# data61/stellar-random-walk

Measured on AMD Instinct MI355X. Metric: walk-steps/sec, higher is better.
Workload: dtype f64

## Files before the change

### include/stellar_rw.h

```cpp
#ifndef STELLAR_RW_H
#define STELLAR_RW_H
#include <stddef.h>
#include <stdint.h>

#ifdef __cplusplus
extern "C" {
#endif

typedef struct srw_handle srw_handle;

enum {
  SRW_OK = 0,
  SRW_ERR_INVALID = 1,
  SRW_ERR_IO = 2,
  SRW_ERR_PARSE = 3,
  SRW_ERR_HIP = 4,
  SRW_ERR_EXISTS = 5,
  SRW_ERR_NOMEM = 6
};

enum {
  SRW_SAMPLER_REFERENCE = 0,
  SRW_SAMPLER_ALIAS = 1
};
enum {
  SRW_RNG_CONST = 0,
  SRW_RNG_PHILOX = 1
};

typedef struct {
  int32_t device;
  int32_t rank;
  int32_t world;
  int32_t flags;
} srw_config;
enum {
  SRW_CFG_OWNER_FROM_PARTITIONS = 1,
  SRW_CFG_COMPACT_IDS = 2,
  SRW_CFG_NO_MEMBERSHIP = 4,
  SRW_CFG_OWNER_HASH_PARTITIONER = 8
};

int32_t srw_create(const srw_config *cfg, srw_handle **out);
void srw_destroy(srw_handle *h);
const char *srw_last_error(const srw_handle *h);
int32_t srw_set_stream(srw_handle *h, void *hip_stream);

int32_t srw_plan_walks(srw_handle *h, int64_t num_walks);

int32_t srw_load_edgelist(srw_handle *h, const char *path, int32_t directed, int32_t weighted,
                          int32_t partitioned, int32_t rdd_partitions);
int32_t srw_load_coo(srw_handle *h, const int32_t *src, const int32_t *dst, const float *w,
                     const int32_t *pid, int64_t n_lines, int32_t directed);
enum { SRW_IDS_I32 = 0, SRW_IDS_I64 = 1 };
int32_t srw_load_coo_device(srw_handle *h, const void *d_src, const void *d_dst, const float *d_w,
                            int64_t n_lines, int32_t id_type, int32_t directed);
int32_t srw_load_adjacency(srw_handle *h, const int32_t *vids, const int64_t *offs, int64_t n_rows,
                           const int32_t *ids, const float *w, const int32_t *pids);
int32_t srw_generate_rmat(srw_handle *h, int32_t scale, int64_t n_edges, uint32_t seed, int32_t weighted,
                          int32_t directed);

int32_t srw_graph_stats(const srw_handle *h, int64_t *n_vertices, int64_t *n_entries);
int32_t srw_graph_vertices(const srw_handle *h, int32_t *out);
int32_t srw_graph_neighbors(const srw_handle *h, int32_t v, int32_t *ids, float *w, int64_t cap, int64_t *n);
int32_t srw_graph_partition(const srw_handle *h, int32_t v, int32_t *pid, int32_t *known);

typedef struct {
  float p, q;
  int32_t walk_length;
  int32_t num_walks;
  int32_t first_walk;
  int32_t rng_mode;
  float const_r;
  uint32_t seed;
  int32_t sampler;
  int32_t flags;
} srw_walk_params;
enum {
  SRW_WALK_FORCE_GENERAL = 1,
  SRW_WALK_NT_LOADS = 2,
  SRW_WALK_CACHED_LOADS = 4,
  SRW_WALK_NO_COMPACT = 16,
  SRW_WALK_NO_PREFIX = 32,
  SRW_WALK_NO_EDGE_HASH = 64,
  SRW_WALK_NO_BINNED = 128,
  SRW_WALK_DEVICE_FORMAT = 131072,
  SRW_WALK_NO_HUB_BITMAPS = 65536,
  SRW_WALK_NO_EDGE_TABLES = 262144,
  SRW_WALK_EDGE_TABLES_ALL = 524288
};

typedef struct {
  int64_t n_walkers;
  int64_t n_steps;
  int64_t dead_ends;
  int64_t sum_deg_curr;
  int64_t sum_deg_prev;
  int64_t ent_reads;
  int64_t fallbacks;
  int64_t trials;
  double kernel_ms;
  int32_t kernel_kind;
  int32_t record_bytes;
  int64_t strategy_steps[12];
  int64_t edge_tables;
  int64_t edge_table_bytes;
  double setup_ms;
} srw_walk_stats;
enum {
  SRW_STRAT_EDGE_TABLE = 0,
  SRW_STRAT_P1 = 1,
  SRW_STRAT_P2 = 2,
  SRW_STRAT_W = 3,
  SRW_STRAT_P3 = 4,
  SRW_STRAT_SCAN = 5,
  SRW_STRAT_PREFIX = 6,
  SRW_STRAT_CHAIN = 7,
  SRW_STRAT_EDGE_MASK = 8,
  SRW_STRAT_Q1_LANE = 9,
  SRW_STAT_HANDED_OVER = 10,
  SRW_STAT_TIES_RESOLVED = 11
};

int32_t srw_walk(srw_handle *h, const srw_walk_params *params, srw_walk_stats *stats);
int32_t srw_walk_to_host(srw_handle *h, const srw_walk_params *params, int32_t *paths, int32_t *lens,
                         srw_walk_stats *stats);
int32_t srw_walk_and_save(srw_handle *h, const srw_walk_params *params, const char *output_dir, int32_t n_parts,
                          int32_t write_crc, srw_walk_stats *stats, int64_t *dead_ends_per_iteration);
int32_t srw_set_sources(srw_handle *h, const int32_t *ids, int64_t n);
int32_t srw_set_sources_device(srw_handle *h, const void *d_ids, int64_t n);
int32_t srw_clear_sources(srw_handle *h);
int32_t srw_sources(const srw_handle *h, int64_t *n);

int32_t srw_vertex_types_set(srw_handle *h, const void *d_types, int64_t n);
int32_t srw_vertex_types(const srw_handle *h, int64_t *n);
int32_t srw_walk_metapath(srw_handle *h, const srw_walk_params *params, const int32_t *pattern, int32_t m, srw_walk_stats *stats);

typedef struct { uint32_t seed; uint32_t epoch; int32_t replace; int32_t flags; } srw_neighbor_params;
enum { SRW_NBR_NO_COMPACT = 1  };
int32_t srw_sample_neighbors(srw_handle *h, const void *d_seeds , int64_t n_seeds,
                             const int32_t *fanouts , int32_t n_layers, const srw_neighbor_params *np,
                             void *const *d_layers , int64_t *n_unknown );

int32_t srw_host_alloc(size_t bytes, void **out);
void srw_host_free(void *p);
int32_t srw_fetch_paths(const srw_handle *h, int32_t *paths, int32_t *lens);
int32_t srw_device_paths(const srw_handle *h, void **d_paths, void **d_lens, int64_t *n_walkers, int32_t *stride);
int32_t srw_write_paths(const srw_handle *h, const char *output_dir, int32_t n_parts, int32_t write_crc);

int32_t srw_alias_row(srw_handle *h, int32_t v, float *prob, int32_t *alias, int64_t cap, int64_t *n, int32_t *regular);

typedef struct {
  int32_t lw;
  int32_t src;
  int32_t prev, curr;
} srw_walker;
typedef struct {
  int32_t lw;
  int32_t v;
} srw_path_ret;
typedef struct { int64_t cap_walkers, cap_rets, chunk_bytes; } srw_shard_layout;
int32_t srw_shard_capacity(const srw_handle *h, int64_t *n_local_vertices, int64_t *n_global_vertices);
int32_t srw_shard_vertex_ranks(const srw_handle *h, int32_t *out);
int32_t srw_shard_layout_for(const srw_handle *h, int32_t batch, double slack, srw_shard_layout *out);
// ... 104 lines not shown
```

### stellar-random-walk_amd/__init__.py

```python
import ctypes as C
import os

import numpy as np

_DIR = os.path.dirname(os.path.abspath(__file__))
LIB_PATH = os.environ.get("SRW_LIB") or os.path.join(_DIR, "libstellar_rw.so")
CLI_PATH = os.path.join(_DIR, "stellar-rw")

OK, ERR_INVALID, ERR_IO, ERR_PARSE, ERR_HIP, ERR_EXISTS, ERR_NOMEM = range(7)
SAMPLER_REFERENCE, SAMPLER_ALIAS = 0, 1
RNG_CONST, RNG_PHILOX = 0, 1
CFG_OWNER_FROM_PARTITIONS = 1
CFG_COMPACT_IDS = 2
CFG_NO_MEMBERSHIP = 4
CFG_OWNER_HASH_PARTITIONER = 8
IDS_I32, IDS_I64 = 0, 1
WALK_FORCE_GENERAL = 1
WALK_NT_LOADS = 2
WALK_CACHED_LOADS = 4
WALK_NO_COMPACT = 16
WALK_NO_PREFIX = 32
WALK_NO_EDGE_HASH = 64
WALK_NO_BINNED = 128
WALK_NO_HUB_BITMAPS = 65536
WALK_DEVICE_FORMAT = 131072
WALK_NO_EDGE_TABLES = 262144
WALK_EDGE_TABLES_ALL = 524288
NBR_NO_COMPACT = 1
NBR_MAX_LAYERS, NBR_MAX_FANOUT, NBR_MAX_DISTINCT_FANOUT = 8, 4096, 64


class W2vParams(C.Structure):
    _fields_ = [("dim", C.c_int32), ("window", C.c_int32), ("iterations", C.c_int32), ("learning_rate", C.c_float),
                ("seed", C.c_uint32), ("threads", C.c_int32)]


def w2v_save(vocab_ids, vectors, output_dir, n_parts=1):
    ids = np.ascontiguousarray(vocab_ids, dtype=np.int32); vec = np.ascontiguousarray(vectors, dtype=np.float32)
    rc = lib().srw_w2v_save(_i32(ids), _f32(vec), len(ids), vec.shape[1] if vec.ndim == 2 else 1, os.fsencode(output_dir), n_parts)
    if rc != 0:
        raise SrwError(rc, "srw_w2v_save: %s" % lib().srw_last_error(None).decode())


class SkipgramParams(C.Structure):
    _fields_ = [("context", C.c_int32), ("num_negatives", C.c_int32), ("seed", C.c_uint32), ("epoch", C.c_uint32)]


class SkipgramBatchParams(C.Structure):
    _fields_ = [("context", C.c_int32), ("num_negatives", C.c_int32), ("seed", C.c_uint32), ("epoch", C.c_uint32),
                ("exclude_window", C.c_int32), ("max_draws", C.c_int32)]


class SgnsParams(C.Structure):
    _fields_ = [("context", C.c_int32), ("num_negatives", C.c_int32), ("dim", C.c_int32), ("center", C.c_int32),
                ("lr", C.c_float), ("reserved", C.c_int32)]


class TopkParams(C.Structure):
    _fields_ = [("dim", C.c_int32), ("k", C.c_int32), ("metric", C.c_int32), ("reserved", C.c_int32)]


TOPK_METRICS = {"cosine": 0, "dot": 1}


class NeighborParams(C.Structure):
    _fields_ = [("seed", C.c_uint32), ("epoch", C.c_uint32), ("replace", C.c_int32), ("flags", C.c_int32)]


class SrwError(RuntimeError):
    def __init__(self, code, msg):
        super().__init__("srw error %d: %s" % (code, msg))
        self.code = code


class Config(C.Structure):
    _fields_ = [("device", C.c_int32), ("rank", C.c_int32), ("world", C.c_int32), ("flags", C.c_int32)]


class WalkParams(C.Structure):
    _fields_ = [("p", C.c_float), ("q", C.c_float), ("walk_length", C.c_int32), ("num_walks", C.c_int32),
                ("first_walk", C.c_int32), ("rng_mode", C.c_int32), ("const_r", C.c_float), ("seed", C.c_uint32),
                ("sampler", C.c_int32), ("flags", C.c_int32)]


class WalkStats(C.Structure):
    _fields_ = [("n_walkers", C.c_int64), ("n_steps", C.c_int64), ("dead_ends", C.c_int64),
                ("sum_deg_curr", C.c_int64), ("sum_deg_prev", C.c_int64), ("ent_reads", C.c_int64),
                ("fallbacks", C.c_int64), ("trials", C.c_int64), ("kernel_ms", C.c_double), ("kernel_kind", C.c_int32),
                ("record_bytes", C.c_int32), ("strategy_steps", C.c_int64 * 12), ("edge_tables", C.c_int64),
                ("edge_table_bytes", C.c_int64), ("setup_ms", C.c_double)]

    def as_dict(self):
        d = {k: getattr(self, k) for k, _ in self._fields_}
        d["strategy_steps"] = dict(zip(STRATEGIES, list(self.strategy_steps)))
        return d


class ShardLayout(C.Structure):
    _fields_ = [("cap_walkers", C.c_int64), ("cap_rets", C.c_int64), ("chunk_bytes", C.c_int64)]


STRATEGIES = ("edge_table", "p1", "p2", "w", "p3", "scan", "prefix", "chain", "edge_mask", "q1_lane", "handed_over_walkers", "ties_resolved")
# ... 333 lines not shown

    def shard_capacity(self):
        a, b = C.c_int64(0), C.c_int64(0)
        self._ck(lib().srw_shard_capacity(self.h, C.byref(a), C.byref(b)))
        return a.value, b.value

    def vertices(self):
        n = self.shard_capacity()[0]
        out = np.zeros(max(n, 1), dtype=np.int32)
        self._ck(lib().srw_graph_vertices(self.h, _i32(out)))
        return out[:n]

    def neighbors(self, v):
        n = C.c_int64(0)
        self._ck(lib().srw_graph_neighbors(self.h, v, None, None, 0, C.byref(n)))
        if n.value < 0:
            return None
        ids = np.zeros(max(n.value, 1), dtype=np.int32)
        w = np.zeros(max(n.value, 1), dtype=np.float32)
        self._ck(lib().srw_graph_neighbors(self.h, v, _i32(ids), _f32(w), n.value, C.byref(n)))
        return ids[:n.value], w[:n.value]

    def partition(self, v):
        pid, known = C.c_int32(0), C.c_int32(0)
        self._ck(lib().srw_graph_partition(self.h, v, C.byref(pid), C.byref(known)))
        return pid.value if known.value else None

    def alias_row(self, v):
        n, reg = C.c_int64(0), C.c_int32(0)
        self._ck(lib().srw_alias_row(self.h, v, None, None, 0, C.byref(n), C.byref(reg)))
        if n.value < 0:
            return None
        prob = np.zeros(max(n.value, 1), dtype=np.float32)
        alias = np.zeros(max(n.value, 1), dtype=np.int32)
        self._ck(lib().srw_alias_row(self.h, v, _f32(prob), _i32(alias), n.value, C.byref(n), C.byref(reg)))
        return reg.value, prob[:n.value], alias[:n.value]

    def set_sources(self, ids):
        if hasattr(ids, "data_ptr") and hasattr(ids, "is_cuda"):
            if "int32" not in str(ids.dtype) or ids.dim() != 1 or not ids.is_contiguous():
                raise TypeError("set_sources: a tensor of ids must be one-dimensional, int32 and contiguous (got %s)" % ids.dtype)
            if ids.is_cuda:
                import torch
                torch.cuda.current_stream(ids.device).synchronize()
                self._ck(lib().srw_set_sources_device(self.h, C.c_void_p(ids.data_ptr()), int(ids.numel())))
                self._src_ids = ids.clone()
                return self
            ids = ids.numpy()
        a = np.asarray(ids)
        if a.size and a.dtype.kind not in "iu":
            raise TypeError("set_sources: vertex ids must be integers (got %s)" % a.dtype)
        if a.size and (int(a.min()) < -2**31 or int(a.max()) > 2**31 - 1):
            raise ValueError("set_sources: a vertex id is outside int32")
        a = np.array(a.reshape(-1), dtype=np.int32)
        self._ck(lib().srw_set_sources(self.h, _i32(a) if a.size else None, a.size))
        self._src_ids = a
        return self

    def clear_sources(self):
        self._ck(lib().srw_clear_sources(self.h))
        self._src_ids = None
        return self

    def sources_len(self):
        n = C.c_int64(0)
        self._ck(lib().srw_sources(self.h, C.byref(n)))
        return None if n.value < 0 else n.value

    def _with_sources(self, sources, call):
        if sources is None:
            return call()
        before = getattr(self, "_src_ids", None) if self.sources_len() is not None else None
        self.set_sources(sources)
        try:
            return call()
        finally:
            if before is None:
                self.clear_sources()
            else:
                self.set_sources(before)

    @staticmethod
    def params(p=1.0, q=1.0, walk_length=80, num_walks=1, first_walk=0, rng="philox", const_r=0.0, seed=42,
               sampler=SAMPLER_REFERENCE, force_general=False, nt_loads=None, occ=0, compact=True, prefix=True, edge_hash=True, binned=True, binned_tune=0, hub_bitmaps=True, device_format=False, edge_tables=True, edge_tables_all=False):
        if sampler == "alias":
            sampler = SAMPLER_ALIAS
        elif sampler == "reference":
            sampler = SAMPLER_REFERENCE
        return WalkParams(np.float32(p), np.float32(q), walk_length, num_walks, first_walk,
                          RNG_CONST if rng == "const" else RNG_PHILOX, np.float32(const_r), seed, sampler,
                          (WALK_FORCE_GENERAL if force_general else 0) | (0 if nt_loads is None else WALK_NT_LOADS if nt_loads else WALK_CACHED_LOADS) | (occ << 8) | (0 if compact else WALK_NO_COMPACT) | (0 if prefix else WALK_NO_PREFIX) | (0 if edge_hash else WALK_NO_EDGE_HASH) | (0 if binned else WALK_NO_BINNED) | (0 if hub_bitmaps else WALK_NO_HUB_BITMAPS) | (WALK_DEVICE_FORMAT if device_format else 0) | (binned_tune << 12) | (0 if edge_tables else WALK_NO_EDGE_TABLES) | (WALK_EDGE_TABLES_ALL if edge_tables_all else 0))

    def walk(self, fetch=True, sources=None, **kw):
        if sources is not None:
            return self._with_sources(sources, lambda: self.walk(fetch=fetch, **kw))
        P = self.params(**kw)
        st = WalkStats()
        self._ck(lib().srw_walk(self.h, C.byref(P), C.byref(st)))
        if not fetch:
            return st.as_dict()
        paths = np.empty((max(st.n_walkers, 1), P.walk_length + 2), dtype=np.int32)
        lens = np.empty(max(st.n_walkers, 1), dtype=np.int32)
        self._ck(lib().srw_fetch_paths(self.h, _i32(paths), _i32(lens)))
        return paths[:st.n_walkers], lens[:st.n_walkers], st.as_dict()

    def set_vertex_types(self, types):
        if types is None:
            self._ck(lib().srw_vertex_types_set(self.h, None, 0))
            return self
        import torch
        mine = getattr(self, "device", None)
        if hasattr(types, "data_ptr") and hasattr(types, "is_cuda"):
            t = types
            if t.dim() != 1:
                raise TypeError("set_vertex_types: types must be one-dimensional [nV] (got %s)" % (tuple(t.shape),))
            if not t.is_contiguous():
                raise TypeError("set_vertex_types: types must be contiguous")
            if str(t.dtype) != "torch.uint8":
                raise TypeError("set_vertex_types: a tensor of types must be torch.uint8 (got %s)" % t.dtype)
            if not t.is_cuda:
                raise TypeError("set_vertex_types: a tensor of types must be in device memory (got %s)" % t.device)
            if mine is not None and t.device.index != mine:
                raise TypeError("set_vertex_types: the tensor must be on the handle's device (cuda:%s), got %s" % (mine, t.device))
        else:
            a = np.asarray(types)
            if a.ndim != 1:
                raise TypeError("set_vertex_types: types must be one-dimensional [nV] (got %s)" % (a.shape,))
            if a.size and a.dtype.kind not in "iu":
                raise TypeError("set_vertex_types: types must be integers (got %s)" % a.dtype)
            if a.size and (int(a.min()) < 0 or int(a.max()) > 255):
                raise TypeError("set_vertex_types: a type is outside the range 0 .. 255")
            t = torch.as_tensor(np.array(a, dtype=np.uint8)).to(torch.device("cuda", mine or 0))
        n = int(t.numel())
        if not n:
            t = torch.zeros(1, dtype=torch.uint8, device=t.device)
        torch.cuda.current_stream(t.device).synchronize()
        self._ck(lib().srw_vertex_types_set(self.h, C.c_void_p(t.data_ptr()), n))
        return self

    def vertex_types_len(self):
        n = C.c_int64(0)
        self._ck(lib().srw_vertex_types(self.h, C.byref(n)))
        return n.value

    @staticmethod
    def _metapath_pattern(pattern):
        if isinstance(pattern, (str, bytes)) or not hasattr(pattern, "__len__"):
            raise TypeError("walk_metapath: pattern must be a sequence of integers (got %s)" % type(pattern).__name__)
        a = np.asarray(pattern)
        if a.ndim != 1 or not 1 <= a.size <= 64:
            raise TypeError("walk_metapath: pattern must have 1 .. 64 entries (got shape %s)" % (a.shape,))
        if a.dtype.kind not in "iu":
            raise TypeError("walk_metapath: pattern entries must be integers (got %s)" % a.dtype)
        if int(a.min()) < -1 or int(a.max()) > 255:
            raise TypeError("walk_metapath: a pattern entry is outside -1 .. 255 (a type, or -1 for any)")
        return np.array(a, dtype=np.int32)

    def walk_metapath(self, pattern, fetch=True, sources=None, **kw):
        pat = self._metapath_pattern(pattern)
        if sources is not None:
            return self._with_sources(sources, lambda: self.walk_metapath(pat, fetch=fetch, **kw))
        P = self.params(**kw)
        st = WalkStats()
        self._ck(lib().srw_walk_metapath(self.h, C.byref(P), _i32(pat), int(pat.size), C.byref(st)))
        if not fetch:
            return st.as_dict()
        paths = np.empty((max(st.n_walkers, 1), P.walk_length + 2), dtype=np.int32)
        lens = np.empty(max(st.n_walkers, 1), dtype=np.int32)
        self._ck(lib().srw_fetch_paths(self.h, _i32(paths), _i32(lens)))
        return paths[:st.n_walkers], lens[:st.n_walkers], st.as_dict()

    @staticmethod
    def _neighbor_fanouts(fanouts, replace):
        if isinstance(fanouts, (str, bytes)) or not hasattr(fanouts, "__len__"):
# ... 612 lines not shown
```

### stellar-random-walk_amd/csrc/walk_kernels.hip

```cpp
#include <algorithm>
#include <map>
#include <tuple>
#include <chrono>
#include <cstring>

#include "engine.h"
#include "sampling.h"
#include "walk_shared.h"

namespace srw {
namespace {
constexpr int TILE = 16;

template <bool NT, int MINW, bool COMPACT>
__global__ __launch_bounds__(TPB, MINW) void k_walk_first_order(GraphView g, const int32_t *__restrict__ verts,
                                                          int64_t n_verts, int64_t n_walkers, int32_t L,
                                                          int32_t first_walk, RngSpec rng,
                                                          int32_t *__restrict__ paths, int32_t *__restrict__ lens,
                                                          DevCounters *ctr) {
  __shared__ int32_t tile[TPB / 64][64][TILE + 1];
  const int lane = lane_id(), wv = threadIdx.x >> 6;
  const int64_t wi = blockIdx.x * (int64_t)TPB + threadIdx.x;
  const int64_t wave_base = wi - lane;
  const int64_t stride = (int64_t)L + 2;
  bool alive = wi < n_walkers;
  uint32_t iter = 0; int32_t src = 0;
  Row r; r.off = 0; r.deg = 0; r.flags = 0;
  if (alive) {
    int64_t it = wi / n_verts, vi = wi - it * n_verts;
    iter = (uint32_t)(first_walk + it);
    src = verts[vi];
    const Row *rp = row_of(g, src);
    if (rp) r = *rp;
  }
  int32_t len = 1;
  unsigned long long reads = 0, dead = 0, fb = 0;
  Bias nobias; nobias.second_order = false; nobias.need_member = false; nobias.p = nobias.q = 1.0f;
  nobias.prev = 0; nobias.prev_sids = nullptr; nobias.prev_deg = 0; nobias.vmin = g.vmin;
  tile[wv][lane][0] = src;
  src = rng_source(g, src);
  for (int32_t s = 1; s <= L + 1; ++s) {
    const int c = s & (TILE - 1);
    int32_t val = -1;
    if (alive) {
      if (r.deg == 0) {
        alive = false; if (s > 1) ++dead;
      } else {
        if (COMPACT && !(r.flags & ROW_IRREGULAR)) {
          const uint32_t m = walk_bits24(rng.seed, iter, (uint32_t)src, (uint32_t)s);
          unsigned rd;
          const CfoEnt e = cfo_pick<NT>(g.cfo + r.off, r.deg, m, rd, g.cfo_reload != 0); reads += rd;
          val = e.id; ++len;
          r.off = (int64_t)(e.link & CFO_NOFF_MASK); r.deg = (int32_t)((e.link >> 40) & 0x7FFFFFu);
          r.flags = (e.link >> 63) ? ROW_IRREGULAR : 0u;
        } else {
          float u = draw_uniform(rng, iter, (uint32_t)src, (uint32_t)s);
          FoEnt e;
          if (r.flags & ROW_IRREGULAR) {
            int32_t k = lane_pick_sequential(g.ent + r.off, r.deg, nobias, u);
            ++fb;
            if (COMPACT) {
              const CfoEnt ce = g.cfo[r.off + k];
              e.id = ce.id; e.noff = (int64_t)(ce.link & CFO_NOFF_MASK); e.ndeg = (int32_t)((ce.link >> 40) & 0x7FFFFFu);
              e.nflags = (ce.link >> 63) ? ROW_IRREGULAR : 0u;
            } else {
              e = g.fo[r.off + k];
            }
          } else {
            unsigned rd; int32_t k;
            e = fo_pick<NT>(g.fo + r.off, r.deg, u, k, rd); reads += rd;
          }
          val = e.id; ++len;
          r.off = e.noff; r.deg = e.ndeg; r.flags = e.nflags;
        }
      }
    }
    tile[wv][lane][c] = val;
    if (c == TILE - 1 || s == L + 1) {
      const int ncols = c + 1;
      const int64_t base_slot = s - c;
      __syncthreads();
#pragma unroll
      for (int rr = 0; rr < 16; ++rr) {
        int row = rr * 4 + (lane >> 4), col = lane & 15;
        int64_t w = wave_base + row;
        if (col < ncols && w < n_walkers) paths[w * stride + base_slot + col] = tile[wv][row][col];
      }
      __syncthreads();
    }
  }
  if (wi < n_walkers) lens[wi] = len;
  flush_counters(ctr, (unsigned long long)(len - 1), dead, 0, 0, reads, fb);
}

__global__ __launch_bounds__(TPB, 4) void k_walk_general(GraphView g, const int32_t *__restrict__ verts,
                                                      int64_t n_verts, int64_t n_walkers, int32_t L,
                                                      int32_t first_walk, RngSpec rng, float p, float q,
                                                      int32_t *__restrict__ paths, int32_t *__restrict__ lens,
                                                      DevCounters *ctr, unsigned long long *cursor, int32_t tune,
                                                      const int32_t *__restrict__ todo, const unsigned long long *todo_n,
                                                      const int32_t *__restrict__ todo_tie, const ChainRec *__restrict__ tie_list,
                                                      const SWalker *__restrict__ tie_out) {
  __shared__ __attribute__((aligned(16))) uint32_t bitmap[TPB / 64][BINNED_LDS_WORDS];
  const int lane = lane_id();
  Member mem; mem.mode = 0; mem.bm = bitmap[threadIdx.x >> 6]; mem.seg_base = 0;
  mem.ehash = g.ehash; mem.ehash_mask = g.ehash_mask;
#ifdef SRW_PHASE_TIMING
  const unsigned long long t_begin = wall_clock64();
#endif
  const int64_t stride = (int64_t)L + 2;
  unsigned long long steps = 0, degc = 0, degp = 0, fb = 0, dead = 0, fast = 0, srch = 0;
  unsigned long long n_strat[12] = {0, 0, 0, 0, 0, 0, 0, 0, 0, 0, 0, 0};
  while (true) {
    unsigned long long grab = 0;
    if (lane == 0) grab = atomicAdd(cursor, 1ull);
    int64_t wi = (int64_t)(((unsigned long long)(uint32_t)__builtin_amdgcn_readfirstlane((int)(grab >> 32)) << 32) |
                           (uint32_t)__builtin_amdgcn_readfirstlane((int)(uint32_t)grab));
    int32_t tie_s = -1, tie_k = 0, tie_next = 0;
    if (todo) {
      if (wi >= (int64_t)*todo_n) break;
      if (todo_tie) {
        const int32_t ci = todo_tie[wi];
        if (ci >= 0) {
          const SWalker o = tie_out[ci];
          if (o.kind == SK_WALKER_RET || o.kind == SK_RET) { tie_s = (int32_t)tie_list[ci].pad; tie_k = o.pad0; tie_next = o.curr; }
        }
      }
      wi = todo[wi];
    } else if (wi >= n_walkers) break;
    int64_t it = wi / n_verts, vi = wi - it * n_verts;
    const uint32_t iter = (uint32_t)(first_walk + it);
    const int32_t src = verts[vi];
    const uint32_t ksrc = (uint32_t)rng_source(g, src);
    int32_t *path = paths + wi * stride;
    if (lane == 0) path[0] = src;
    int32_t prev = src, curr = src, len = 1;
    Row rprev; rprev.off = 0; rprev.deg = 0; rprev.flags = 0;
    int64_t eprev = 0;
    for (int32_t s = 1; s <= L + 1; ++s) {
      const bool second = s > 1;
      const int64_t cslot = (int64_t)curr - g.vmin;
      const bool in_range = cslot >= 0 && cslot < g.n_slots;
      const bool want_tab = g.eb_off && second && q != 1.0f && !(tune & 16);
      Row r = g.rows[in_range ? cslot : 0];
      uint32_t eo = EB_NONE;
      if (want_tab) eo = g.eb_off[eprev];
      if (!in_range) { r.off = 0; r.deg = 0; r.flags = 0; }
      if (r.deg == 0) { dead += s > 1; break; }
      Bias b;
      b.p = p; b.q = q; b.prev = prev; b.second_order = second; b.need_member = second && (q != 1.0f); b.vmin = g.vmin;
      b.prev_sids = g.sids + rprev.off; b.prev_deg = rprev.deg; b.prev_hub = rprev.flags >> ROW_HUB_SHIFT;
      float u = draw_uniform(rng, iter, ksrc, (uint32_t)s);
      unsigned f = 0, sv = 0;
#ifdef SRW_PHASE_TIMING
      mem.t_step0 = wall_clock64();
#endif
      SRW_T0(mem);
      int32_t k = -1, next = 0;
      bool binned_served = false, have_next = false;
      unsigned which = SRW_STRAT_SCAN;
      if (s == tie_s) { k = tie_k; next = tie_next; have_next = true; binned_served = true; which = SRW_STRAT_EDGE_TABLE; f = 1; n_strat[SRW_STAT_TIES_RESOLVED] += 1; }
      else if (want_tab) {
        if (r.deg <= g.eb_mask_max) {
          if (r.deg <= 32 || eo != EB_NONE) {
            k = wave_pick_masked(g, r, b, eo, r.deg > 32 ? g.em_bits + (size_t)eo * 4 : nullptr, u, f, next);
            have_next = true; binned_served = true; which = SRW_STRAT_EDGE_MASK;
            srch += 8ull * (unsigned long long)r.deg + 4ull * (unsigned long long)((r.deg + 31) >> 5);
          }
        } else if (eo != EB_NONE && (r.flags & ROW_PQ_OK)) {
          k = wave_pick_edge_table(g, r, b, g.eb_bins + (size_t)eo * 8, u, f, sv, mem, next, mem.bm + 2 * BIN_CAP);
          if (k >= 0) { have_next = true; binned_served = true; which = SRW_STRAT_EDGE_TABLE; srch += 8ull * EB_BINS; }
// ... 527 lines not shown
    fprintf(stderr, "[handover] walkers %llu | q1 reasons: irregular row %llu, non-positive sum %llu, boundary draw %llu\n",
            c.strat[SRW_STAT_HANDED_OVER], c.why[0], c.why[1], c.why[2]);
  if (!stats) return;
  stats->n_steps = (int64_t)c.steps; stats->dead_ends = (int64_t)c.dead_ends;
  stats->sum_deg_curr = (int64_t)c.sum_deg_curr; stats->sum_deg_prev = (int64_t)c.sum_deg_prev;
  stats->ent_reads = (int64_t)c.ent_reads; stats->fallbacks = (int64_t)c.fallbacks; stats->trials = (int64_t)c.trials;
  for (int i = 0; i < 12; ++i) stats->strategy_steps[i] = (int64_t)c.strat[i];
  stats->edge_tables = (h->g.has_eb && h->g.use_eb) ? h->g.eb_tables : 0;
  stats->edge_table_bytes = (h->g.has_eb && h->g.use_eb) ? h->g.eb_bytes : 0;
}

void check_params(const srw_walk_params &P) {
  if (P.walk_length < 0) throw Error(SRW_ERR_INVALID, "walk_length must be >= 0");
  if (P.num_walks < 0) throw Error(SRW_ERR_INVALID, "num_walks must be >= 0");
  if (P.rng_mode != SRW_RNG_CONST && P.rng_mode != SRW_RNG_PHILOX) throw Error(SRW_ERR_INVALID, "bad rng_mode");
  if (P.sampler != SRW_SAMPLER_REFERENCE && P.sampler != SRW_SAMPLER_ALIAS) throw Error(SRW_ERR_INVALID, "bad sampler");
  if (P.sampler == SRW_SAMPLER_ALIAS && P.rng_mode != SRW_RNG_PHILOX)
    throw Error(SRW_ERR_INVALID, "Mode A draws several uniforms per step: it needs SRW_RNG_PHILOX");
}

namespace {
struct LaunchInfo { int kind; int record_bytes; };

struct StreamDrain {
  srw_handle *h;
  explicit StreamDrain(srw_handle *hh) : h(hh) {}
  ~StreamDrain() {
    if (h->copy_stream) (void)hipStreamSynchronize(h->copy_stream);
    if (h->stream) (void)hipStreamSynchronize(h->stream);
  }
};

__global__ void k_paths_to_ids(int32_t *__restrict__ paths, const int32_t *__restrict__ lens, int64_t n_walkers, int64_t stride,
                               const int32_t *__restrict__ orig_id) {
  const int lane = lane_id();
  for (int64_t w = blockIdx.x * (int64_t)(TPB / 64) + (threadIdx.x >> 6); w < n_walkers; w += (int64_t)gridDim.x * (TPB / 64)) {
    const int32_t len = lens[w];
    int32_t *row = paths + w * stride;
    for (int32_t k = lane; k < len; k += 64) row[k] = orig_id[row[k]];
  }
}

}

void paths_to_ids(srw_handle *h, int32_t *d_paths, const int32_t *d_lens, int64_t n_walkers, int64_t stride) {
  const int64_t nb = std::min<int64_t>((n_walkers + TPB / 64 - 1) / (TPB / 64), (int64_t)h->n_cus * 32);
  hipLaunchKernelGGL(k_paths_to_ids, dim3((unsigned)nb), dim3(TPB), 0, h->stream, d_paths, d_lens, n_walkers, stride, (const int32_t *)h->g.orig_id.p);
  SRW_HIP(hipGetLastError());
}

namespace {
LaunchInfo launch_walk(srw_handle *h, const srw_walk_params &P, int32_t num_walks, int32_t first_walk, int32_t *d_paths,
                       int32_t *d_lens) {
  Graph &g = h->g;
  { const char *e = getenv("SRW_DEBUG_CHAIN_DEG"); g.dbg_chain_deg = e && *e ? atoi(e) : 0; }
  hipStream_t st = h->stream;
  const int32_t *verts = h->start_verts();
  const int64_t n_verts = h->walkers_per_iteration();
  const int64_t n_walkers = (int64_t)num_walks * n_verts;
  const bool alias = P.sampler == SRW_SAMPLER_ALIAS;
  bool first_order_compact = false;
  const bool first_order = !alias && (P.p == 1.0f && P.q == 1.0f) && !(P.flags & SRW_WALK_FORCE_GENERAL);
  RngSpec rng; rng.mode = P.rng_mode; rng.const_r = P.const_r; rng.seed = P.seed;
  GraphView gv = g.view();
  if (alias) {
    int64_t blocks = (n_walkers + TPB - 1) / TPB;
    const size_t al_bytes = (size_t)g.n_entries * sizeof(AEnt);
    (void)al_bytes;
    const bool nt = (P.flags & SRW_WALK_NT_LOADS) != 0;
    if (nt)
      hipLaunchKernelGGL(k_walk_alias<true>, dim3((unsigned)blocks), dim3(TPB), 0, st, gv, verts, n_verts, n_walkers,
                         P.walk_length, first_walk, P.seed, P.p, P.q, d_paths, d_lens, h->counters.p);
    else
      hipLaunchKernelGGL(k_walk_alias<false>, dim3((unsigned)blocks), dim3(TPB), 0, st, gv, verts, n_verts, n_walkers,
                         P.walk_length, first_walk, P.seed, P.p, P.q, d_paths, d_lens, h->counters.p);
  } else if (first_order) {
    int64_t blocks = (n_walkers + TPB - 1) / TPB;
    const size_t fo_bytes = (size_t)g.n_entries * sizeof(FoEnt);
    const bool nt = (P.flags & SRW_WALK_NT_LOADS) ? true
                    : (P.flags & SRW_WALK_CACHED_LOADS) ? false : fo_bytes > ((size_t)2 << 30);
    const int occ = (P.flags >> 8) & 0xF;
    const bool compact = g.has_cfo && P.rng_mode == SRW_RNG_PHILOX && !(P.flags & SRW_WALK_NO_COMPACT);
    first_order_compact = compact;
#define SRW_LAUNCH_FO(NTV, MW, CP)                                                                                  \
  hipLaunchKernelGGL((k_walk_first_order<NTV, MW, CP>), dim3((unsigned)blocks), dim3(TPB), 0, st, gv, verts,           \
                     n_verts, n_walkers, P.walk_length, first_walk, rng, d_paths, d_lens, h->counters.p)
    if (compact) {
      const bool ntc = (P.flags & SRW_WALK_NT_LOADS) ? true : (P.flags & SRW_WALK_CACHED_LOADS) ? false
                       : (size_t)g.n_entries * sizeof(CfoEnt) > ((size_t)2 << 30);
      if (ntc) SRW_LAUNCH_FO(true, 1, true); else SRW_LAUNCH_FO(false, 1, true);
    } else if (nt) { if (occ == 8) SRW_LAUNCH_FO(true, 8, false); else if (occ == 7) SRW_LAUNCH_FO(true, 7, false); else SRW_LAUNCH_FO(true, 1, false); }
    else    { if (occ == 8) SRW_LAUNCH_FO(false, 8, false); else if (occ == 7) SRW_LAUNCH_FO(false, 7, false); else SRW_LAUNCH_FO(false, 1, false); }
#undef SRW_LAUNCH_FO
  } else {
    int64_t blocks = std::min<int64_t>((n_walkers * 64 + TPB - 1) / TPB, (int64_t)h->n_cus * 8);
    h->walk_cursor.ensure(2);
    SRW_HIP(hipMemsetAsync(h->walk_cursor.p, 0, 2 * sizeof(unsigned long long), st));
    const int32_t tune = (int32_t)(((P.flags >> 12) & 15) | ((P.flags & SRW_WALK_NO_BINNED) ? 16 : 0));
    const bool lean = gv.eb_off && g.eb_complete && P.q != 1.0f && tune == 0 && !getenv("SRW_NO_LEAN_KERNEL");
    const bool q1 = P.q == 1.0f && P.p != 1.0f && P.rng_mode == SRW_RNG_PHILOX && g.has_cfo && g.has_pq && g.has_rev &&
                    g.pq_bad_rows == 0 && tune == 0 && !(P.flags & SRW_WALK_NO_PREFIX) && !getenv("SRW_NO_Q1_KERNEL");
    const int32_t *todo = nullptr;
    const int32_t *todo_tie = nullptr; const ChainRec *tie_list = nullptr; const SWalker *tie_out = nullptr;
    TieSink tie; tie.hdr = nullptr; tie.recs = nullptr; tie.list = nullptr; tie.cur = nullptr; tie.todo_tie = nullptr;
    ChainBufs cb;
    const bool ties = lean && P.rng_mode == SRW_RNG_PHILOX && !getenv("SRW_NO_TIE_KERNELS");
    if (q1 || lean) h->walk_todo.ensure(2 * (size_t)n_walkers);
    if (ties) {
      cb = chain_bufs(h);
      SRW_HIP(hipMemsetAsync(cb.tie_cur, 0, 48, st));
      SRW_HIP(hipMemsetAsync(cb.tie_out, 0xFF, (size_t)CHAIN_CAP * sizeof(SWalker), st));
      tie.hdr = cb.tie_hdr; tie.recs = cb.tie_recs; tie.list = cb.list; tie.cur = cb.tie_cur + 2;
      tie.todo_tie = h->walk_todo.p + n_walkers;
    }
    auto resolve_ties = [&]() {
      if (!ties) return;
      ShardIO io; io.recv = reinterpret_cast<const char *>(cb.tie_hdr); io.chunk_bytes = 0; io.cap_w = CHAIN_CAP; io.cap_r = 0;
      io.world = 1; io.rank = 0; io.batch = 0x7FFFFFFF; io.pt = nullptr; io.lens = nullptr; io.n_rows = 0;
      srw_walk_params Pc = P; Pc.first_walk = first_walk;
      static const int n_pass = getenv("SRW_TIE_PASSES") ? std::max(1, atoi(getenv("SRW_TIE_PASSES"))) : 8;
      for (int pass = 0; pass < n_pass; ++pass)
        enqueue_chain(h, cb, gv, io, Pc, 0, 0, rng, cb.tie_out, -1, cb.tie_cur, cb.tie_skip, cb.tie_cur + 3);
      todo_tie = tie.todo_tie; tie_list = cb.list; tie_out = cb.tie_out;
    };
    if (q1) {
      const int64_t qb = (n_walkers + TPB - 1) / TPB;
      const uint32_t q1_max_ret = getenv("SRW_Q1_MAX_RET") ? (uint32_t)atoi(getenv("SRW_Q1_MAX_RET")) : 16u;
      if ((size_t)g.n_entries * sizeof(CfoEnt) > ((size_t)2 << 30))
        hipLaunchKernelGGL(k_walk_q1<true>, dim3((unsigned)qb), dim3(TPB), 0, st, gv, verts, n_verts, n_walkers, P.walk_length,
                           first_walk, rng, P.p, d_paths, d_lens, h->counters.p, h->walk_todo.p, h->walk_cursor.p + 1, q1_max_ret);
      else
        hipLaunchKernelGGL(k_walk_q1<false>, dim3((unsigned)qb), dim3(TPB), 0, st, gv, verts, n_verts, n_walkers, P.walk_length,
                           first_walk, rng, P.p, d_paths, d_lens, h->counters.p, h->walk_todo.p, h->walk_cursor.p + 1, q1_max_ret);
      todo = h->walk_todo.p;
    }
    if (lean) {
      int64_t lb = std::min<int64_t>((n_walkers * 64 + TPB - 1) / TPB, (int64_t)h->n_cus * 16);
      TabArgs ta;
      ta.g = gv; ta.verts = verts; ta.n_verts = n_verts; ta.n_walkers = n_walkers; ta.L = P.walk_length; ta.first_walk = first_walk;
      ta.rng = rng; ta.p = P.p; ta.q = P.q; ta.paths = d_paths; ta.lens = d_lens; ta.ctr = h->counters.p; ta.cursor = h->walk_cursor.p;
      ta.todo = h->walk_todo.p; ta.todo_n = h->walk_cursor.p + 1; ta.tie = tie;
      const int lanes = getenv("SRW_TABLE_LANES") ? atoi(getenv("SRW_TABLE_LANES")) : (gv.ebp.min_sh <= 6 ? 2 : -1);
      if (lanes >= 0) {
        launch_walk_tables_lanes(ta, gv.bf_off != nullptr, lanes, getenv("SRW_LANE_CSH") ? atoi(getenv("SRW_LANE_CSH")) : 6, h->n_cus, st);
      } else if (gv.bf_off) {
        hipLaunchKernelGGL((k_walk_tables<true>), dim3((unsigned)lb), dim3(TPB), 0, st, ta);
      } else {
        hipLaunchKernelGGL((k_walk_tables<false>), dim3((unsigned)lb), dim3(TPB), 0, st, ta);
      }
      SRW_HIP(hipMemsetAsync(h->walk_cursor.p, 0, sizeof(unsigned long long), st));
      todo = h->walk_todo.p;
      resolve_ties();
    }
    hipLaunchKernelGGL(k_walk_general, dim3((unsigned)blocks), dim3(TPB), 0, st, gv, verts, n_verts, n_walkers,
                       P.walk_length, first_walk, rng, P.p, P.q, d_paths, d_lens, h->counters.p, h->walk_cursor.p, tune, todo,
                       h->walk_cursor.p + 1, todo_tie, tie_list, tie_out);
  }
  SRW_HIP(hipGetLastError());
  LaunchInfo li;
  li.kind = alias ? 3 : first_order ? 1 : 2;
  li.record_bytes = first_order_compact ? 16 : (first_order || alias) ? 32 : 0;
  if (g.compact && n_walkers > 0) paths_to_ids(h, d_paths, d_lens, n_walkers, (int64_t)P.walk_length + 2);
  return li;
}

void prepare_tables(srw_handle *h, const srw_walk_params &P) {
  const bool timing = getenv("SRW_TIMING") != nullptr;
  auto t_phase = std::chrono::steady_clock::now();
  auto phase = [&](const char *name) {
    if (!timing) return;
    (void)hipStreamSynchronize(h->stream);
    const auto t = std::chrono::steady_clock::now();
    const double ms = std::chrono::duration<double, std::milli>(t - t_phase).count();
    if (ms >= 20.0) fprintf(stderr, "[timing] prepare_tables: %s %.0f ms\n", name, ms);
    t_phase = t;
  };
// ... 453 lines not shown
```

Baseline: 42.25 billion.

## Flush first-order walk paths in 64-byte-aligned chunks per walker within each wave

The first-order walk kernel used to stage path steps in an LDS tile and write them out every 16 steps, using block-wide __syncthreads. That spilled path rows across misaligned 64-byte segments. The new default path tracks each walker's row alignment and flushes whenever that walker's output reaches a 16-int (64-byte) boundary. Each flush uses a wave-level ballot and wave barriers in place of block barriers, with four rows written per pass. This should cut partial-line writes and block synchronisation, at the cost of more frequent, irregular flush loops and extra index arithmetic. The old scheme stays available behind a legacy flag.

```diff
diff --git a/include/stellar_rw.h b/include/stellar_rw.h
--- a/include/stellar_rw.h
+++ b/include/stellar_rw.h
@@ -80,6 +80,7 @@
   SRW_WALK_FORCE_GENERAL = 1,
   SRW_WALK_NT_LOADS = 2,
   SRW_WALK_CACHED_LOADS = 4,
+  SRW_WALK_LEGACY_FLUSH = 8,
   SRW_WALK_NO_COMPACT = 16,
   SRW_WALK_NO_PREFIX = 32,
   SRW_WALK_NO_EDGE_HASH = 64,
diff --git a/stellar-random-walk_amd/__init__.py b/stellar-random-walk_amd/__init__.py
--- a/stellar-random-walk_amd/__init__.py
+++ b/stellar-random-walk_amd/__init__.py
@@ -18,6 +18,7 @@
 WALK_FORCE_GENERAL = 1
 WALK_NT_LOADS = 2
 WALK_CACHED_LOADS = 4
+WALK_LEGACY_FLUSH = 8
 WALK_NO_COMPACT = 16
 WALK_NO_PREFIX = 32
 WALK_NO_EDGE_HASH = 64
@@ -517,14 +518,14 @@
 
     @staticmethod
     def params(p=1.0, q=1.0, walk_length=80, num_walks=1, first_walk=0, rng="philox", const_r=0.0, seed=42,
-               sampler=SAMPLER_REFERENCE, force_general=False, nt_loads=None, occ=0, compact=True, prefix=True, edge_hash=True, binned=True, binned_tune=0, hub_bitmaps=True, device_format=False, edge_tables=True, edge_tables_all=False):
+               sampler=SAMPLER_REFERENCE, force_general=False, nt_loads=None, occ=0, compact=True, prefix=True, edge_hash=True, binned=True, binned_tune=0, hub_bitmaps=True, device_format=False, edge_tables=True, edge_tables_all=False, legacy_flush=False):
         if sampler == "alias":
             sampler = SAMPLER_ALIAS
         elif sampler == "reference":
             sampler = SAMPLER_REFERENCE
         return WalkParams(np.float32(p), np.float32(q), walk_length, num_walks, first_walk,
                           RNG_CONST if rng == "const" else RNG_PHILOX, np.float32(const_r), seed, sampler,
-                          (WALK_FORCE_GENERAL if force_general else 0) | (0 if nt_loads is None else WALK_NT_LOADS if nt_loads else WALK_CACHED_LOADS) | (occ << 8) | (0 if compact else WALK_NO_COMPACT) | (0 if prefix else WALK_NO_PREFIX) | (0 if edge_hash else WALK_NO_EDGE_HASH) | (0 if binned else WALK_NO_BINNED) | (0 if hub_bitmaps else WALK_NO_HUB_BITMAPS) | (WALK_DEVICE_FORMAT if device_format else 0) | (binned_tune << 12) | (0 if edge_tables else WALK_NO_EDGE_TABLES) | (WALK_EDGE_TABLES_ALL if edge_tables_all else 0))
+                          (WALK_FORCE_GENERAL if force_general else 0) | (0 if nt_loads is None else WALK_NT_LOADS if nt_loads else WALK_CACHED_LOADS) | (occ << 8) | (0 if compact else WALK_NO_COMPACT) | (0 if prefix else WALK_NO_PREFIX) | (0 if edge_hash else WALK_NO_EDGE_HASH) | (0 if binned else WALK_NO_BINNED) | (0 if hub_bitmaps else WALK_NO_HUB_BITMAPS) | (WALK_DEVICE_FORMAT if device_format else 0) | (binned_tune << 12) | (0 if edge_tables else WALK_NO_EDGE_TABLES) | (WALK_EDGE_TABLES_ALL if edge_tables_all else 0) | (WALK_LEGACY_FLUSH if legacy_flush else 0))
 
     def walk(self, fetch=True, sources=None, **kw):
         if sources is not None:
diff --git a/stellar-random-walk_amd/csrc/walk_kernels.hip b/stellar-random-walk_amd/csrc/walk_kernels.hip
--- a/stellar-random-walk_amd/csrc/walk_kernels.hip
+++ b/stellar-random-walk_amd/csrc/walk_kernels.hip
@@ -12,7 +12,7 @@
 namespace {
 constexpr int TILE = 16;
 
-template <bool NT, int MINW, bool COMPACT>
+template <bool NT, int MINW, bool COMPACT, bool LEGACY>
 __global__ __launch_bounds__(TPB, MINW) void k_walk_first_order(GraphView g, const int32_t *__restrict__ verts,
                                                           int64_t n_verts, int64_t n_walkers, int32_t L,
                                                           int32_t first_walk, RngSpec rng,
@@ -38,6 +38,9 @@
   Bias nobias; nobias.second_order = false; nobias.need_member = false; nobias.p = nobias.q = 1.0f;
   nobias.prev = 0; nobias.prev_sids = nullptr; nobias.prev_deg = 0; nobias.vmin = g.vmin;
   tile[wv][lane][0] = src;
+  const uint32_t pbase = (uint32_t)(reinterpret_cast<uintptr_t>(paths) >> 2);
+  const uint32_t a_own = (pbase + (uint32_t)wi * (uint32_t)stride) & (TILE - 1);
+  if (!LEGACY && wi < n_walkers && a_own == TILE - 1) paths[wi * stride] = src;
   src = rng_source(g, src);
   for (int32_t s = 1; s <= L + 1; ++s) {
     const int c = s & (TILE - 1);
@@ -76,17 +79,44 @@
       }
     }
     tile[wv][lane][c] = val;
-    if (c == TILE - 1 || s == L + 1) {
-      const int ncols = c + 1;
-      const int64_t base_slot = s - c;
-      __syncthreads();
+    if constexpr (LEGACY) {
+      if (c == TILE - 1 || s == L + 1) {
+        const int ncols = c + 1;
+        const int64_t base_slot = s - c;
+        __syncthreads();
 #pragma unroll
-      for (int rr = 0; rr < 16; ++rr) {
-        int row = rr * 4 + (lane >> 4), col = lane & 15;
-        int64_t w = wave_base + row;
-        if (col < ncols && w < n_walkers) paths[w * stride + base_slot + col] = tile[wv][row][col];
-      }
-      __syncthreads();
+        for (int rr = 0; rr < 16; ++rr) {
+          int row = rr * 4 + (lane >> 4), col = lane & 15;
+          int64_t w = wave_base + row;
+          if (col < ncols && w < n_walkers) paths[w * stride + base_slot + col] = tile[wv][row][col];
+        }
+        __syncthreads();
+      }
+    } else {
+      const bool due = wi < n_walkers && ((((a_own + (uint32_t)s) & (TILE - 1)) == TILE - 1) || s == L + 1);
+      unsigned long long todo = __ballot(due);
+      if (todo) {
+        __builtin_amdgcn_fence(__ATOMIC_RELEASE, "wavefront");
+        __builtin_amdgcn_wave_barrier();
+        const int grp = lane / TILE, col = lane & (TILE - 1);
+        do {
+          int row = -1;
+#pragma unroll
+          for (int k = 0; k < 64 / TILE; ++k) {
+            const int b = todo ? (int)__builtin_ctzll(todo) : -1;
+            todo &= todo - 1;
+            if (grp == k) row = b;
+          }
+          if (row >= 0) {
+            const int64_t w = wave_base + row;
+            const uint32_t a = (pbase + (uint32_t)w * (uint32_t)stride) & (TILE - 1);
+            const int32_t t = s - (int32_t)((a + (uint32_t)s) & (TILE - 1)) + col;
+            if (t >= 0 && t <= s) paths[w * stride + t] = tile[wv][row][t & (TILE - 1)];
+          }
+        } while (todo);
+        __builtin_amdgcn_fence(__ATOMIC_ACQUIRE, "wavefront");
+        __builtin_amdgcn_wave_barrier();
+      }
     }
   }
   if (wi < n_walkers) lens[wi] = len;
@@ -780,9 +810,12 @@
     const int occ = (P.flags >> 8) & 0xF;
     const bool compact = g.has_cfo && P.rng_mode == SRW_RNG_PHILOX && !(P.flags & SRW_WALK_NO_COMPACT);
     first_order_compact = compact;
+    const bool legacy_flush = (P.flags & SRW_WALK_LEGACY_FLUSH) != 0;
+#define SRW_LAUNCH_FO_W(NTV, MW, CP, LG)                                                                            \
+  hipLaunchKernelGGL((k_walk_first_order<NTV, MW, CP, LG>), dim3((unsigned)blocks), dim3(TPB), 0, st, gv, verts,       \
+                     n_verts, n_walkers, P.walk_length, first_walk, rng, d_paths, d_lens, h->counters.p)
 #define SRW_LAUNCH_FO(NTV, MW, CP)                                                                                  \
-  hipLaunchKernelGGL((k_walk_first_order<NTV, MW, CP>), dim3((unsigned)blocks), dim3(TPB), 0, st, gv, verts,           \
-                     n_verts, n_walkers, P.walk_length, first_walk, rng, d_paths, d_lens, h->counters.p)
+  do { if (legacy_flush) SRW_LAUNCH_FO_W(NTV, MW, CP, true); else SRW_LAUNCH_FO_W(NTV, MW, CP, false); } while (0)
     if (compact) {
       const bool ntc = (P.flags & SRW_WALK_NT_LOADS) ? true : (P.flags & SRW_WALK_CACHED_LOADS) ? false
                        : (size_t)g.n_entries * sizeof(CfoEnt) > ((size_t)2 << 30);
@@ -790,6 +823,7 @@
     } else if (nt) { if (occ == 8) SRW_LAUNCH_FO(true, 8, false); else if (occ == 7) SRW_LAUNCH_FO(true, 7, false); else SRW_LAUNCH_FO(true, 1, false); }
     else    { if (occ == 8) SRW_LAUNCH_FO(false, 8, false); else if (occ == 7) SRW_LAUNCH_FO(false, 7, false); else SRW_LAUNCH_FO(false, 1, false); }
 #undef SRW_LAUNCH_FO
+#undef SRW_LAUNCH_FO_W
   } else {
     int64_t blocks = std::min<int64_t>((n_walkers * 64 + TPB - 1) / TPB, (int64_t)h->n_cus * 8);
     h->walk_cursor.ensure(2);
```

Result: faster. 43.10 billion, median of 6 (+2.0%).
